# tprodanov/locityper

Hardware: AMD Instinct MI355X
Metric: reads/s through the whole genotyping path (scored + prefiltered + default solver scheme); reads_scored_per_s and genotypes_solved_per_s give the two halves (higher is better)
Workload: dtype f64

## Files before the change

locityper_amd/csrc/lcty_api.hip:

```cpp
#include <algorithm>
#include <cmath>
#include <memory>
#include <numeric>

#include "lcty_objects.hpp"

using namespace lcty;

namespace lcty {
static thread_local std::string g_last_error;
thread_local hipStream_t tl_stream = nullptr;
void set_last_error(const std::string& msg) { g_last_error = msg; }
}

hipEvent_t lcty_ctx::get_event() {
    hipEvent_t e;
    if (!event_pool.empty()) { e = event_pool.back(); event_pool.pop_back(); return e; }
    LCTY_HIP(hipEventCreate(&e));
    return e;
}

void lcty_ctx::fold_oldest(lcty::KernelTimer& t, size_t count) {
    count = std::min(count, t.pending.size());
    for (size_t i = 0; i < count; i++) {
        float ms = 0.f;
        LCTY_HIP(hipEventSynchronize(t.pending[i].second));
        LCTY_HIP(hipEventElapsedTime(&ms, t.pending[i].first, t.pending[i].second));
        t.total_ms += ms; t.launches++;
        event_pool.push_back(t.pending[i].first); event_pool.push_back(t.pending[i].second);
    }
    t.pending.erase(t.pending.begin(), t.pending.begin() + static_cast<std::ptrdiff_t>(count));
}

extern "C" {

int32_t lcty_ctx_set_knob(lcty_ctx* ctx, const char* name, int64_t value) {
    return guarded([&] {
        if (!ctx || !name) fail(LCTY_ERR_INVALID_INPUT, "null argument");
        static const char* const known[] = {"transfer_levels", "transfer_scratch_mb", "transfer_waves", "transfer_cap_new", "transfer_arena",
                                            "depth_table_start", "solve_budget_mb", "solve_chains_per_wave", "solve_extra_start", "solve_lds_weights",
                                            "anneal_lds_weights", "contig_info_slide", "gather_chunk_mb", "prefilter_gram", "prefilter_gram_cols",
                                            "prefilter_gram_levels", "comm_fail_at", "score_lean", "arena_cap_pct", "exact_threads", "host_threads",
                                            "score_lean_keep", "score_lean_two", "queue_early_head", "db_chunk_cols", "basis_batch_words",
                                            "align_batch_pairs", "align_hash_bits", "align_dp_cells", "align_match_budget", "align_cigar_store_mb", "pafvcf_hash_bits", "pafvcf_table_mb",
                                            "genome_max_bases", "sample_bam_hash_bits", "sample_bam_max_slice_bytes", "sample_bam_inflate",
                                            "bgzf_deflate", "bgzf_deflate_max_bytes", "aln_bam_max_slice_bytes", "vcf_max_slice_bytes", "fastx_window_bytes", "fastx_window_limit", "recruit_blocks",
                                            "recruited_init_units", "recruited_max_bytes",
#ifdef LCTY_DIAG
                                            "solve_stats", "queue_trace", "map_trace", "exact_trace", "solve_greedy_form", "solve_anneal_timing", "score_timing",
                                            "solve_init_tiles", "transfer_phases", "genome_scan_form",
#endif
                                            nullptr};
        bool ok = false;
        for (const char* const* k = known; *k; k++) ok |= strcmp(*k, name) == 0;
        if (!ok) fail(LCTY_ERR_INVALID_INPUT, "unknown knob '%s'", name);
        if (strcmp(name, "bgzf_deflate") == 0 && value != 0 && value != 1) fail(LCTY_ERR_INVALID_INPUT, "bgzf_deflate = %lld (0: host, 1: device)", static_cast<long long>(value));
        if (value < 0) ctx->knobs.erase(name); else ctx->knobs[name] = value;
    });
}

int32_t lcty_ctx_set_path(lcty_ctx* ctx, const char* name, const char* path) {
    return guarded([&] {
        if (!ctx || !name) fail(LCTY_ERR_INVALID_INPUT, "null argument");
        if (strcmp(name, "exact_dump") != 0) fail(LCTY_ERR_INVALID_INPUT, "unknown path '%s'", name);
        ctx->exact_dump_path = path ? path : "";
    });
}

const char* lcty_last_error(void) { return g_last_error.c_str(); }
const char* lcty_version(void) { return "locityper_hip 0.1.0 (gfx950)"; }

int32_t lcty_device_count(void) {
    int n = 0;
    if (hipGetDeviceCount(&n) != hipSuccess) { (void)hipGetLastError(); return 0; }
    return n;
}

int32_t lcty_ctx_create(int32_t device_id, lcty_ctx** out) {
    return guarded([&] {
        if (!out) fail(LCTY_ERR_INVALID_INPUT, "null argument");
        int n = 0;
        if (hipGetDeviceCount(&n) != hipSuccess || n == 0) {
            (void)hipGetLastError();
            fail(LCTY_ERR_RUNTIME, "no HIP device is visible: liblocityper_hip has no CPU fallback");
        }
        if (device_id < 0 || device_id >= n) fail(LCTY_ERR_INVALID_INPUT, "device %d out of range (0..%d)", device_id, n - 1);
        auto c = std::unique_ptr<lcty_ctx>(new lcty_ctx());
        c->device = device_id;
        LCTY_HIP(hipSetDevice(device_id));
// ... 327 lines not shown
```

locityper_amd/csrc/lcty_solve_device.hpp:

```cpp
#pragma once
#include "lcty_objects.hpp"

namespace lcty {

constexpr uint32_t MAXP = 4;
constexpr uint32_t NONE32S = 0xFFFFFFFFu;
constexpr uint32_t MID_NONE24 = 0xFFFFFFu;
constexpr uint64_t WINDOW_KEY_XOR = 0xD1B54A32D192ED03ull;
constexpr uint64_t INIT_KEY_XOR = 0x8CB92BA72F3D8DD7ull;

struct FastDiv {
    uint32_t d, m, s1, s2;
    __host__ static FastDiv make(uint32_t d) {
        FastDiv f{d, 0, 0, 0};
        uint32_t l = 0;
        while ((1ull << l) < d) l++;
        f.m = static_cast<uint32_t>(((1ull << 32) * ((1ull << l) - d)) / d + 1);
        f.s1 = l < 1 ? l : 1; f.s2 = l > 0 ? l - 1 : 0;
        return f;
    }
    __device__ __forceinline__ uint32_t div(uint32_t n) const {
        const uint32_t t = __umulhi(m, n);
        return (t + ((n - t) >> s1)) >> s2;
    }
// ... 124 lines not shown
static_assert(sizeof(InitGroup) == 48 && INIT_TILE_R <= 8, "InitGroup layout");
struct InitPlan {
    std::vector<InitGroup> groups; std::vector<InitChainP> chains;
    uint32_t T = 0, R = 0;
    size_t lds = 0;
};

inline void set_rec_list(SolveView& V, uint64_t n_reads) {
    V.seg_reads = static_cast<uint32_t>(((n_reads + INIT_SEGS - 1) / INIT_SEGS + 63) / 64 * 64);
    if (V.seg_reads == 0) V.seg_reads = 64;
    V.rstride = static_cast<uint64_t>(INIT_SEGS) * V.seg_reads;
}
inline size_t init_chain_lds(uint32_t wstride) { return ((static_cast<size_t>(wstride) * 4 + 15) & ~static_cast<size_t>(15)) + 256 * 8 + 64; }

template <typename... P, typename... A>
void launch_lds(lcty_ctx* ctx, int timer, void (*kernel)(P...), dim3 grid, dim3 block, size_t lds, hipStream_t s, const A&... args) {
    if (lds > 48 * 1024)
        LCTY_HIP(hipFuncSetAttribute(reinterpret_cast<const void*>(kernel), hipFuncAttributeMaxDynamicSharedMemorySize, static_cast<int>(lds)));
    auto go = [&] { hipLaunchKernelGGL(kernel, grid, block, lds, s, args...); };
    if (timer < 0) go();
    else ctx->timed(timer, go, s);
    LCTY_HIP(hipGetLastError());
}

void check_solver(const lcty_solver* solver);

void ensure_solver_tables(lcty_reads* reads);
void ensure_depth_table(lcty_locus* loc, uint64_t want);
void build_depth_table_into(const lcty_locus* loc, uint32_t depth, DevBuf<double>& out, hipStream_t s);
bool solver_lds_fits(uint32_t wstride);
struct InitHost {
    const uint16_t* genotypes; const uint64_t* seeds; const uint16_t* row_of; const lcty_locus* loc; uint32_t n_cus;
    uint32_t lds_budget;
};
void plan_init_groups(const SolveView& V, const InitHost& H, uint32_t nch, InitPlan& plan);
void launch_init(lcty_ctx* ctx, const SolveView& V, uint32_t nch, size_t lds_init, hipStream_t s, const InitHost* host, lcty_ctx::SolveWorkspace& ws,
                 InitPlan& plan);
void launch_greedy_chains(lcty_ctx* ctx, SolveView& V, uint32_t nch, hipStream_t stream, lcty_ctx::SolveWorkspace& ws);
void launch_anneal(lcty_ctx* ctx, const SolveView& V, uint32_t nch, hipStream_t s);
void launch_pause(hipStream_t s);
void launch_store_cur(ChainRec* recs, const uint32_t* words, uint64_t n, hipStream_t s);
void launch_pack_rows_count(uint64_t n, const LocCell* table, uint64_t ngp, uint32_t n_good, const uint16_t* alleles, uint32_t n_rows,
                            unsigned long long* total, hipStream_t s);
void launch_pack_rows(uint64_t n, const LocCell* table, const uint32_t* table_ext, const double* table_unm, uint64_t ngp, uint32_t n_good,
                      const uint16_t* alleles, uint32_t n_rows, const PairAlnDev* pa, LocEntry* cells, uint64_t out_stride, PairAlnDev* extras,
                      unsigned long long* cursor, hipStream_t s);
void launch_place_rows(uint64_t n, const LocEntry* cells, uint64_t in_stride, uint32_t n_good, uint32_t n_rows, uint32_t ext_base, LocCell* full,
                       uint32_t* full_ext, double* full_unm, bool write_unm, uint64_t full_stride, uint64_t first, hipStream_t s);
void launch_pad_rows(uint64_t n, LocCell* full, uint32_t* full_ext, double* full_unm, uint64_t full_stride, uint64_t from, uint32_t n_rows, hipStream_t s);
void launch_count_unexplained(uint32_t blocks, const uint8_t* status, const double* unmapped, const double* matrix, uint64_t n_pairs, uint32_t A,
                              const uint16_t* ids, uint32_t ploidy, unsigned long long* out, hipStream_t s);
void launch_read_nw(const SolveView& V, uint32_t* nw, hipStream_t s);
void launch_assignment_counts(const SolveView& V, const uint32_t* nw, const uint64_t* read_off, uint16_t* counts, hipStream_t s);

}
```

locityper_amd/csrc/lcty_solve_host.hip:

```cpp
#include <algorithm>
#include <atomic>
#include <cmath>
#include <exception>
#include <memory>
#include <numeric>
#include <future>
#include <thread>
#include <type_traits>

#include "lcty_exact.hpp"
#include "lcty_solve_device.hpp"

using namespace lcty;

namespace {

double students_t_cdf(double freedom, double x) {
    if (std::isinf(freedom)) return 0.5 * std::erfc(-x / std::sqrt(2.0));
    const double h = freedom / (freedom + x * x);
    const double ib = 0.5 * math::beta_reg(freedom / 2.0, 0.5, h);
    return x <= 0.0 ? ib : 1.0 - ib;
}

double compare_two(double mean1, double var1, uint32_t att1, double mean2, double var2, uint32_t att2) {
// ... 18 lines not shown

void sort_by_mean(const double* lik_mean, uint64_t* ixs, uint64_t n) {
    std::sort(ixs, ixs + n, [&](uint64_t a, uint64_t b) {
        if (lik_mean[a] != lik_mean[b]) return lik_mean[a] > lik_mean[b];
        return a < b;
    });
}

double ln_sum(const double* v, size_t n) {
    if (n == 0) return -std::numeric_limits<double>::infinity();
    if (n == 1) return v[0];
    double m = -std::numeric_limits<double>::infinity();
    for (size_t i = 0; i < n; i++) m = std::fmax(m, v[i]);
    if (std::isinf(m)) return m;
    double s = 0.0;
    for (size_t i = 0; i < n; i++) s += std::exp(v[i] - m);
    return m + std::log(s);
}

}

namespace {

struct StageRunner {
    lcty_reads* reads; lcty_ctx* ctx; lcty_locus* loc;
    SolveView V{};
    uint64_t n_gt; uint32_t ploidy, attempts;
    size_t lds_init = 0;
    uint64_t gt_per_batch = 1, depth_cap = 2;
    uint32_t lane;
    hipStream_t stream;
    lcty_ctx::SolveWorkspace& ws;
    InitPlan init_plan;
    InitHost init_host{nullptr, nullptr, nullptr, nullptr, 0, 0};
    const RowGatherer* gathered_rows = nullptr;

    StageRunner(lcty_reads* r, const uint16_t* genotypes, uint64_t n_gt_, uint32_t ploidy_, const lcty_solver* solver, uint32_t attempts_,
                const uint64_t* chain_seeds, uint32_t lane_ = 0, const RowGatherer* gathered = nullptr)
        : reads(r), n_gt(n_gt_), ploidy(ploidy_), attempts(attempts_), lane(lane_), ws(check_args(r, genotypes, solver, chain_seeds, lane_)) {
        if (!reads->scored) fail(LCTY_ERR_INVALID_INPUT, "lcty_score_reads has not been called on this batch");
        if (ploidy == 0 || ploidy > MAXP) fail(LCTY_ERR_UNSUPPORTED, "the device solver handles ploidy 1..%u", MAXP);
        if (attempts == 0) fail(LCTY_ERR_INVALID_INPUT, "At least one attempt is required for each stage");
        check_solver(solver);
        ctx = reads->ctx; loc = reads->locus; gathered_rows = gathered;
        ctx->activate();
        stream = lane ? ctx->side_stream() : ctx->stream;
        reads->check_device_error(stream);
        const uint32_t A = loc->n_alleles;
        for (uint64_t i = 0; i < n_gt * ploidy; i++)
            if (genotypes[i] >= A) fail(LCTY_ERR_INVALID_INPUT, "genotype refers to allele %u >= %u", genotypes[i], A);
        if (n_gt * attempts >= 0x7FFFFFFFull) fail(LCTY_ERR_UNSUPPORTED, "too many chains in one stage");
        if (!gathered) ensure_solver_tables(reads);
        reads->stat_chains = reads->stat_iterations = reads->stat_accepted = 0;
        const uint64_t n_good = gathered ? gathered->n_good : reads->n_good_cached, ngp = gathered ? gathered->ngp : reads->ngp;
        uint32_t min_w = 0xFFFFFFFFu;
        for (uint32_t a = 0; a < A; a++) min_w = std::min(min_w, std::max(loc->n_windows[a], 1u));
        depth_cap = 2 * n_good + 2;
        uint64_t first_width = std::min<uint64_t>(4 * n_good / min_w + 64, depth_cap);
        if (ctx->knob("depth_table_start", 0) > 0)
            first_width = static_cast<uint64_t>(ctx->knob("depth_table_start", 0));
        ensure_depth_table(loc, first_width);

        V.by_window = FastDiv::make(loc->bg.window); V.by_tweak = FastDiv::make(2 * static_cast<uint32_t>(loc->prm.tweak) + 1);
        V.A = A; V.window = loc->bg.window; V.left_padding = loc->left_padding; V.tweak = static_cast<uint32_t>(loc->prm.tweak);
        V.min_weight = loc->prm.min_weight; V.prob_diff = loc->prm.prob_diff;
        V.depth_contrib = 1.0 + loc->prm.lik_skew; V.aln_contrib = 1.0 - loc->prm.lik_skew;
        V.n_windows = loc->d_n_windows.p; V.reg_start = loc->d_reg_start.p; V.allele_len = loc->d_allele_len.p;
// ... 255 lines not shown
            std::vector<uint32_t> words(V.rstride);
            for (size_t k = 0; k < gn; k++) {
                Held& h = held[k];
                const uint32_t c0 = todo[g0 + k];
                for (uint64_t j = 0; j < V.rstride; j++) words[j] = h.recs[j].rp_cur;
                for (uint32_t i = 0; i < h.model.n; i++) words[h.place[i]] = (words[h.place[i]] & 0xFFFFFFu) | (static_cast<uint32_t>(h.res.assign[i]) << 24);
                d_words.upload(words.data(), V.rstride, s);
                const uint32_t c1 = shared_model ? std::min(c0 + attempts, nch) : c0 + 1;
                for (uint32_t c = c0; c < c1; c++) {
                    if (nnt[c] != h.model.n) fail(LCTY_ERR_RUNTIME, "exact solver: the attempts of a genotype without a tweak differ in their models");
                    launch_store_cur(V.recs + static_cast<uint64_t>(c) * V.rstride, d_words.p, V.rstride, s);
                    liks[c] = pri[c / attempts] + h.res.value;
                    parts[4ull * c] = h.res.aln_lik; parts[4ull * c + 1] = h.res.depth_lik; parts[4ull * c + 2] = static_cast<double>(h.res.nodes); parts[4ull * c + 3] = 0.0;
                }
                LCTY_HIP(hipStreamSynchronize(s));
            }
            LCTY_HIP(hipStreamSynchronize(s));
        }
        ws.liks.upload(liks.data(), nch, s);
        ws.parts.upload(parts.data(), 4ull * nch, s);
        LCTY_HIP(hipStreamSynchronize(s));
    }

    template <typename F>
    void run(const uint16_t* genotypes, const double* priors, const uint64_t* chain_seeds, F&& after_batch) {
        hipStream_t s = stream;
        std::vector<double> liks(gt_per_batch * attempts);
        for (uint64_t g0 = 0; g0 < n_gt;) {
            const uint64_t ng = std::min(gt_per_batch, n_gt - g0), nch = ng * attempts;
            bool smaller_batches = false;
            upload_genotypes(genotypes + g0 * ploidy, ng);
            ws.seeds.upload(chain_seeds + g0 * attempts, nch, s);
            init_host = InitHost{genotypes + g0 * ploidy, chain_seeds + g0 * attempts, gathered_rows ? gathered_rows->row_of.data() : nullptr, loc,
                                 static_cast<uint32_t>(ctx->props.multiProcessorCount), lane == 1 ? 32u * 1024u : 0u};
            if (priors) ws.pri.upload(priors + g0, ng, s);
            V.priors = priors ? ws.pri.p : nullptr;
            for (;;) {
                V.lut = loc->d_lut_ext.p; V.lut_depth = loc->lut_ext_depth; V.lut_shift = static_cast<uint32_t>(__builtin_ctz(loc->lut_ext_depth));
                launch(static_cast<uint32_t>(nch));
                uint32_t ovf[2] = {0, 0};
                ws.ovf.download(ovf, 2, s);
                ws.liks.download(liks.data(), nch, s);
                LCTY_HIP(hipStreamSynchronize(s));
                if (!ovf[0]) {
                    std::vector<double> parts(4 * nch);
                    ws.parts.download(parts.data(), 4 * nch, s);
                    LCTY_HIP(hipStreamSynchronize(s));
                    double sum = 0, mx = 0, mn = 1e300, acc = 0;
                    for (uint64_t c = 0; c < nch; c++) {
                        const double it = parts[4 * c + 2];
                        sum += it; mx = std::max(mx, it); mn = std::min(mn, it); acc += parts[4 * c + 3];
                    }
                    reads->stat_chains += nch; reads->stat_iterations += static_cast<uint64_t>(sum);
                    reads->stat_accepted += static_cast<uint64_t>(acc);
                    if (ctx->diag_knob("solve_stats", 0))
                        fprintf(stderr, "[lcty solve] chains=%llu iterations mean=%.0f min=%.0f max=%.0f accepted mean=%.0f lut_depth=%u\n",
                                static_cast<unsigned long long>(nch), sum / nch, mn, mx, acc / nch, loc->lut_ext_depth);
                    break;
                }
                if (ovf[0] == 2) fail(LCTY_ERR_UNSUPPORTED, "a read pair with more than 255 possible locations on one genotype (or 2^24 further locations in a chain)");
                if (ovf[0] == 3) fail(LCTY_ERR_RUNTIME, "annealing kernel: the staging wavefront and the chain lost each other");
                ws.ovf.zero(s);
                if (ovf[0] == 4) {
                    if (ovf[1] >= (1u << 24)) fail(LCTY_ERR_UNSUPPORTED, "2^24 or more further locations in one chain");
                    ws.extra_cap = std::min<uint32_t>(std::max<uint32_t>(ovf[1] + ovf[1] / 8 + 64, 2 * ws.extra_cap), (1u << 24) - 1);
                    const uint64_t before = gt_per_batch;
                    plan_batches();
// ... 694 lines not shown
```

locityper_amd/csrc/lcty_solve_kernels.hip:

```cpp
#include <algorithm>
#include <cmath>
#include <type_traits>
#include <vector>

#include "lcty_solve_device.hpp"

namespace lcty {


__global__ __launch_bounds__(256) void build_loc_table_kernel(const uint32_t* __restrict__ good_ix, uint32_t n_good, uint64_t ngp,
                                                              uint32_t A, const uint32_t* __restrict__ pa_idx,
                                                              const uint64_t* __restrict__ pa_off, const PairAlnDev* __restrict__ pa,
                                                              const double* __restrict__ unmapped, LocCell* __restrict__ table,
                                                              uint32_t* __restrict__ table_ext, double* __restrict__ table_unm,
                                                              uint32_t* __restrict__ err) {
    __shared__ LocCell tile[32][33];
    __shared__ uint32_t tile_ext[32][33];
    const uint32_t g0 = blockIdx.x * 32, c0 = blockIdx.y * 32;
    const uint32_t tx = threadIdx.x & 31u, ty = threadIdx.x >> 5;
    if (blockIdx.y == 0 && threadIdx.x < 32) {
        const uint32_t g = g0 + threadIdx.x;
        if (g < ngp) table_unm[g] = g < n_good ? unmapped[good_ix[g]] : 0.0;
    }
    for (uint32_t i = ty; i < 32; i += 8) {
// ... 388 lines not shown
    __syncthreads();
    const uint32_t ex_total = seg_cnt[4];
    if (tid == 0) {
        if (ex_total > V.extra_cap) { atomicMax(V.overflow, 4u); atomicMax(V.overflow + 1, ex_total); }
        if (ex_total >= (1u << 24)) atomicMax(V.overflow, 2u);
    }
    for (uint32_t s = 128; s > 0; s >>= 1) {
        if (tid < s) red[tid] += red[tid + s];
        __syncthreads();
    }
    uint32_t* gdepth = V.c_depth + static_cast<uint64_t>(chain) * V.wstride;
    for (uint32_t w = tid; w < G.total_w; w += 256) gdepth[w] = depth[w];
    if (tid == 0) {
        uint32_t* cum = V.c_seg + static_cast<uint64_t>(chain) * 4;
        uint32_t run = 0;
        for (uint32_t k = 0; k < INIT_SEGS; k++) { cum[k] = run; run += seg_cnt[k]; }
        V.c_aln[chain] = red[0]; V.c_nnt[chain] = run; V.c_totw[chain] = G.total_w;
    }
}

__device__ __forceinline__ uint64_t counter_fin(uint64_t z) {
    z = (z ^ (z >> 30)) * 0xbf58476d1ce4e5b9ull;
    z = (z ^ (z >> 27)) * 0x94d049bb133111ebull;
    return z ^ (z >> 31);
}
constexpr uint64_t GOLDEN64 = 0x9e3779b97f4a7c15ull;
typedef uint32_t u32x4_t __attribute__((ext_vector_type(4)));
__device__ __forceinline__ void store_16(uint4* p, uint4 v) {
    u32x4_t x; x.x = v.x; x.y = v.y; x.z = v.z; x.w = v.w;
    __builtin_nontemporal_store(x, reinterpret_cast<u32x4_t*>(p));
}
__host__ __device__ inline size_t init_tile_lds(uint32_t T, uint32_t R, uint32_t wstride) {
    const size_t depth = (static_cast<size_t>(T) * wstride * 4 + 15) & ~static_cast<size_t>(15);
    return depth + static_cast<size_t>(T) * 256 * 8 + 4ull * R * 64 * 16 + static_cast<size_t>(T) * 4 * 8 + static_cast<size_t>(T) * 4 * 5 + 64;
}

__device__ __forceinline__ void init_tile_deferred(const SolveView& V, const InitChainP* __restrict__ cp, uint32_t T, uint32_t* depth, double* aln_def,
                                                   uint32_t* ex_cnt, unsigned long long* queue, uint32_t head, uint32_t n, uint32_t wave, uint32_t lane, bool random_start) {
    double add = 0.0;
    uint32_t my_c = 0xFFFFFFFFu;
    if (lane < n) {
        const unsigned long long packed = __hip_atomic_load(&queue[(head + lane) & (INIT_TILE_Q - 1)], __ATOMIC_RELAXED, __HIP_MEMORY_SCOPE_WORKGROUP);
        const uint2 item = make_uint2(static_cast<uint32_t>(packed), static_cast<uint32_t>(packed >> 32));
        const uint32_t c = item.x >> 24, rp = item.x & 0xFFFFFFu, slot = item.y;
        const InitChainP P = cp[c];
        Geno<2> G;
        G.id[0] = P.id0; G.id[1] = P.id1; G.row[0] = P.row0; G.row[1] = P.row1; G.shift[0] = P.shift0; G.shift[1] = P.shift1;
        G.reg_start[0] = P.rs0; G.reg_start[1] = P.rs1; G.reg_end[0] = P.re0; G.reg_end[1] = P.re1; G.total_w = P.total_w;
        Locs<2> L;
        locs_init<2>(L, V, rp, G);
        if (L.nw > 255) atomicMax(V.overflow, 2u);
        uint32_t a0 = 0;
        if (L.nw > 1 && random_start)
            a0 = static_cast<uint32_t>(__umul64hi(counter_u64(P.seed ^ INIT_KEY_XOR, rp), static_cast<uint64_t>(L.nw)));
        const uint32_t nloc = min(L.nw, 255u), n_extra = nloc > 2 ? nloc - 2u : 0u;
        uint32_t eix = 0;
        if (n_extra) eix = atomicAdd(&ex_cnt[c], n_extra);
        const bool room = static_cast<uint64_t>(eix) + n_extra <= V.extra_cap;
        ExtraLoc* extra = V.extra + static_cast<uint64_t>(P.chain) * V.extra_cap;
        ChainRec rec; rec.rp_cur = rp | (a0 << 24); rec.meta = nloc | (eix << 8);
        rec.lp0 = rec.lp1 = 0.0; rec.win0 = rec.win1 = 0;
        LocIter<2> it; it.start(L);
        LocOut o;
        for (uint32_t t = 0; t < nloc && it.next(L, V, o); t++) {
            uint32_t wa, wb;
            loc_windows(V, G, o, P.seed, rp, t, &wa, &wb);
            const uint32_t win = wa | (wb << 16);
// ... 2 lines not shown
            else if (room) { ExtraLoc e; e.lp = o.lp; e.win = win; e._pad = 0; extra[eix + t - 2] = e; }
            if (t == a0) {
                atomicAdd(&depth[static_cast<size_t>(c) * V.wstride + wa], 1u);
                atomicAdd(&depth[static_cast<size_t>(c) * V.wstride + wb], 1u);
                add = o.lp;
                my_c = c;
            }
        }
        if (L.nw > 1) V.recs[static_cast<uint64_t>(P.chain) * V.rstride + static_cast<uint64_t>(wave) * V.seg_reads + slot] = rec;
    }
    for (uint32_t c = 0; c < T; c++) {
        unsigned long long m = __ballot(my_c == c);
        if (!m) continue;
        double acc = aln_def[c * 4 + wave];
        while (m) {
            const int l = __ffsll(static_cast<long long>(m)) - 1;
            acc += __hiloint2double(__builtin_amdgcn_readlane(__double2hiint(add), l), __builtin_amdgcn_readlane(__double2loint(add), l));
            m &= m - 1;
        }
        if (lane == 0) aln_def[c * 4 + wave] = acc;
    }
}

__global__ __launch_bounds__(256) void solve_init_tile_kernel(const SolveView V, const InitGroup* __restrict__ groups, const InitChainP* __restrict__ chains,
                                                             unsigned long long* lists, const uint32_t T_max, const uint32_t R_max) {
    extern __shared__ __align__(16) uint8_t smem[];
    const uint32_t tid = threadIdx.x, lane = tid & 63u, wave = __builtin_amdgcn_readfirstlane(tid >> 6);
    const InitGroup& grp = groups[blockIdx.x];
    const uint32_t T = grp.n_chains, R = grp.n_rows;
    const InitChainP* __restrict__ cp = chains + grp.first;
    const uint32_t W = V.wstride;
    uint32_t* depth = reinterpret_cast<uint32_t*>(smem);
    size_t at = (static_cast<size_t>(T_max) * W * 4 + 15) & ~static_cast<size_t>(15);
    double* aln = reinterpret_cast<double*>(smem + at); at += static_cast<size_t>(T_max) * 256 * 8;
    uint4* stage = reinterpret_cast<uint4*>(smem + at) + static_cast<size_t>(wave) * R_max * 64; at += 4ull * R_max * 64 * 16;
    unsigned long long* queue = lists + (static_cast<size_t>(blockIdx.x) * 4 + wave) * INIT_TILE_Q;
    double* aln_def = reinterpret_cast<double*>(smem + at); at += static_cast<size_t>(T_max) * 4 * 8;
    uint32_t* ex_cnt = reinterpret_cast<uint32_t*>(smem + at); at += static_cast<size_t>(T_max) * 4;
    uint32_t* seg_cnt = reinterpret_cast<uint32_t*>(smem + at);

    for (uint32_t c = 0; c < T; c++) {
        const InitChainP P = cp[c];
        double* ww = V.c_ww + static_cast<uint64_t>(P.chain) * W;
        uint8_t* wgc = V.c_gc + static_cast<uint64_t>(P.chain) * W;
        uint32_t* wuc = V.n_wk ? V.c_uc + static_cast<uint64_t>(P.chain) * W : nullptr;
        for (uint32_t w = tid; w < P.total_w; w += 256) {
            depth[c * W + w] = 0;
            double weight = 0.0; uint32_t g = 0, uc = V.n_wk - 1;
            if (w >= 2) {
                const bool second = w >= P.shift1;
                const uint32_t allele = second ? P.id1 : P.id0, sh = second ? P.shift1 : P.shift0, rs = second ? P.rs1 : P.rs0;
                const uint32_t start = rs + (w - sh) * V.window, end = start + V.window;
                const uint32_t left = min(V.tweak, start), right = min(V.tweak, V.allele_len[allele] - end);
                const uint64_t r = counter_u64(P.seed ^ WINDOW_KEY_XOR, w);
                const int64_t off = -static_cast<int64_t>(left) + static_cast<int64_t>(__umul64hi(r, static_cast<uint64_t>(left + right + 1)));
                const uint32_t wstart = static_cast<uint32_t>(static_cast<int64_t>(start) + off);
                const uint32_t i = V.ci_off[allele] + (wstart > V.left_padding ? wstart - V.left_padding : 0u);
                weight = V.win_weight[i];
                g = V.gc[i];
                if (wuc) uc = V.uniq_cnt[i] | (static_cast<uint32_t>(V.compl_cnt[i]) << 16);
                if (weight < V.min_weight || weight < 1e-7) { weight = 0.0; g = 0; uc = V.n_wk - 1; }
            }
            ww[w] = weight; wgc[w] = static_cast<uint8_t>(g);
            if (wuc) wuc[w] = uc;
        }
        aln[c * 256 + tid] = 0.0;
        if (tid < 4) aln_def[c * 4 + tid] = 0.0;
        if (tid == 0) ex_cnt[c] = 0;
    }
    __syncthreads();

    const bool random_start = V.solver.kind == LCTY_SOLVER_ANNEAL || (V.solver.kind == LCTY_SOLVER_GREEDY && !V.solver.best_start);
    const uint32_t seg_lo = min(wave * V.seg_reads, V.n_good), seg_hi = min(seg_lo + V.seg_reads, V.n_good);
    uint64_t row_at[INIT_TILE_R];
#pragma unroll
    for (uint32_t r = 0; r < INIT_TILE_R; r++) row_at[r] = static_cast<uint64_t>(grp.row[r < R ? r : 0]) * V.ngp;
    const uint4* __restrict__ table = reinterpret_cast<const uint4*>(V.table);
    uint4 nxt[INIT_TILE_R]; double nxt_unm = 0.0;
#pragma unroll
    for (uint32_t r = 0; r < INIT_TILE_R; r++) nxt[r] = make_uint4(0, 0, 0, 0);
    if (seg_lo + lane < seg_hi) {
#pragma unroll
        for (uint32_t r = 0; r < INIT_TILE_R; r++) if (r < R) nxt[r] = table[row_at[r] + seg_lo + lane];
        nxt_unm = V.table_unm[seg_lo + lane];
    }
    uint32_t n_recs_all = 0;
    uint32_t qn = 0, qhead = 0;
    for (uint32_t base = seg_lo; base < seg_hi; base += 64) {
        const uint32_t rp = base + lane;
        const bool in = rp < seg_hi;
#pragma unroll
        for (uint32_t r = 0; r < INIT_TILE_R; r++) if (r < R) stage[r * 64 + lane] = nxt[r];
        const double unm = nxt_unm;
        if (rp + 64 < seg_hi) {
#pragma unroll
            for (uint32_t r = 0; r < INIT_TILE_R; r++) if (r < R) nxt[r] = table[row_at[r] + rp + 64];
            nxt_unm = V.table_unm[rp + 64];
        }
        const uint64_t zbase = ((static_cast<uint64_t>(rp) << 16) + 1ull) * GOLDEN64;
        const uint64_t abase = (static_cast<uint64_t>(rp) + 1ull) * GOLDEN64;
        for (uint32_t c = 0; c < T; c++) {
            const InitChainP P = cp[c];
            const uint4 qa = stage[P.ia * 64 + lane], qb = stage[P.ib * 64 + lane];
            const double aln_before = aln[c * 256 + tid];
            const double lpA = __hiloint2double(static_cast<int>(qa.y), static_cast<int>(qa.x));
            const double lpB = __hiloint2double(static_cast<int>(qb.y), static_cast<int>(qb.x));
            const uint32_t rawA = qa.z >> 24, rawB = qb.z >> 24;
            const double thresh = fmax(fmax(lpA, lpB), unm) - V.prob_diff;
            const bool kA = in && rawA != 0 && lpA >= thresh, kB = in && rawB != 0 && lpB >= thresh, kU = in && unm >= thresh;
            const bool multi = (kA && rawA > 1) || (kB && rawB > 1);
            const uint32_t nw = (kA ? 1u : 0u) + (kB ? 1u : 0u) + (kU ? 1u : 0u);
            bool nontrivial = nw > 1;
            if (__any(multi && nw == 1)) {
                if (multi && nw == 1) {
                    const uint32_t ext = V.table_ext[static_cast<uint64_t>(kA ? P.row0 : P.row1) * V.ngp + rp];
                    nontrivial = V.pa[ext].ln_prob >= thresh;
                }
            }
            const unsigned long long nt_mask = __ballot(nontrivial);
            const uint32_t before = __builtin_amdgcn_readlane(n_recs_all, c);
            const uint32_t slot = before + static_cast<uint32_t>(__popcll(nt_mask & ((1ull << lane) - 1ull)));
            {
                const uint32_t after = __builtin_amdgcn_readfirstlane(before + static_cast<uint32_t>(__popcll(nt_mask)));
                uint32_t m0_was;
                asm volatile("s_mov_b32 %1, m0\n\ts_mov_b32 m0, %3\n\tv_writelane_b32 %0, %2, m0\n\ts_mov_b32 m0, %1"
                             : "+v"(n_recs_all), "=&s"(m0_was) : "s"(after), "s"(c));
            }
            const unsigned long long mm = __ballot(multi);
            if (mm) {
                if (multi)
                    __hip_atomic_store(&queue[(qhead + qn + static_cast<uint32_t>(__popcll(mm & ((1ull << lane) - 1ull)))) & (INIT_TILE_Q - 1)],
                                       static_cast<unsigned long long>(rp | (c << 24)) | (static_cast<unsigned long long>(slot) << 32), __ATOMIC_RELAXED,
                                       __HIP_MEMORY_SCOPE_WAVEFRONT);
                qn += static_cast<uint32_t>(__popcll(mm));
            }
            const bool BgtA = lpB > lpA, UgtA = unm > lpA, UgtB = unm > lpB;
            const uint32_t posA = ((kB && BgtA) ? 1u : 0u) + ((kU && UgtA) ? 1u : 0u);
// ... 2 lines not shown
            if (V.tweak) {
                const uint64_t z0 = P.seed + zbase;
                const uint64_t rA = counter_fin(z0 + (posA == 0 ? 0ull : posA == 1 ? GOLDEN64 : 2ull * GOLDEN64));
                const uint64_t rB = counter_fin(z0 + (posB == 0 ? 0ull : posB == 1 ? GOLDEN64 : 2ull * GOLDEN64));
                tA1 = V.by_tweak.mod(static_cast<uint32_t>(rA >> 32)); tA2 = V.by_tweak.mod(static_cast<uint32_t>(rA));
                tB1 = V.by_tweak.mod(static_cast<uint32_t>(rB >> 32)); tB2 = V.by_tweak.mod(static_cast<uint32_t>(rB));
            }
            auto window_ix = [&](uint32_t mid, bool none, uint32_t tw, uint32_t rs, uint32_t re, uint32_t sh) -> uint32_t {
                const uint32_t m = mid + tw;
                uint32_t q = V.by_window.div(m - rs) + sh;
                asm volatile("" : "+v"(q));
                const uint32_t inside = (rs <= m && m < re) ? q : 1u;
                return none ? 0u : inside;
            };
            const uint32_t midA1 = qa.z & MID_NONE24, midB1 = qb.z & MID_NONE24;
            const uint32_t winA = window_ix(midA1, midA1 == MID_NONE24, tA1, P.rs0, P.re0, P.shift0) |
                                  (window_ix(qa.w, qa.w == NONE32S, tA2, P.rs0, P.re0, P.shift0) << 16);
            const uint32_t winB = window_ix(midB1, midB1 == MID_NONE24, tB1, P.rs1, P.re1, P.shift1) |
                                  (window_ix(qb.w, qb.w == NONE32S, tB2, P.rs1, P.re1, P.shift1) << 16);
            const bool a_0 = kA && posA == 0, b_0 = kB && posB == 0, a_1 = kA && posA == 1, b_1 = kB && posB == 1, a_2 = kA && posA == 2, b_2 = kB && posB == 2;
            const double lp0 = a_0 ? lpA : (b_0 ? lpB : unm), lp1 = a_1 ? lpA : (b_1 ? lpB : unm), lp2 = a_2 ? lpA : (b_2 ? lpB : unm);
            const uint32_t win0 = a_0 ? winA : (b_0 ? winB : 0u), win1 = a_1 ? winA : (b_1 ? winB : 0u), win2 = a_2 ? winA : (b_2 ? winB : 0u);
            uint32_t a0 = 0;
            double lps = lp0; uint32_t wins = win0;
            if (random_start) {
                const uint64_t r = counter_fin((P.seed ^ INIT_KEY_XOR) + abase);
                a0 = nw > 1 ? static_cast<uint32_t>(__umul64hi(r, static_cast<uint64_t>(nw))) : 0u;
                lps = a0 == 0 ? lp0 : (a0 == 1 ? lp1 : lp2); wins = a0 == 0 ? win0 : (a0 == 1 ? win1 : win2);
            }
            const bool fast = !multi && nw != 0;
            if (fast) {
                atomicAdd(&depth[c * W + (wins & 0xFFFFu)], 1u);
                atomicAdd(&depth[c * W + (wins >> 16)], 1u);
                aln[c * 256 + tid] = aln_before + lps;
            }
            uint32_t eix = 0;
            if (fast && nw == 3) {
                eix = atomicAdd(&ex_cnt[c], 1u);
                if (eix < V.extra_cap) {
                    ExtraLoc e; e.lp = lp2; e.win = win2; e._pad = 0;
                    V.extra[static_cast<uint64_t>(P.chain) * V.extra_cap + eix] = e;
                }
            }
            if (fast && nw > 1) {
                uint4* dst = reinterpret_cast<uint4*>(V.recs + static_cast<uint64_t>(P.chain) * V.rstride + static_cast<uint64_t>(wave) * V.seg_reads + slot);
                store_16(dst, make_uint4(rp | (a0 << 24), nw | (eix << 8), static_cast<uint32_t>(__double2loint(lp0)), static_cast<uint32_t>(__double2hiint(lp0))));
                store_16(dst + 1, make_uint4(static_cast<uint32_t>(__double2loint(lp1)), static_cast<uint32_t>(__double2hiint(lp1)), win0, win1));
            }
        }
        const bool last = base + 64 >= seg_hi;
        if (qn >= 64 || (last && qn)) {
            __builtin_amdgcn_fence(__ATOMIC_RELEASE, "workgroup");
            __builtin_amdgcn_wave_barrier();
            __builtin_amdgcn_fence(__ATOMIC_ACQUIRE, "workgroup");
            while (qn >= 64 || (last && qn)) {
                const uint32_t n = min(qn, 64u);
                init_tile_deferred(V, cp, T, depth, aln_def, ex_cnt, queue, qhead, n, wave, lane, random_start);
                qhead = (qhead + n) & (INIT_TILE_Q - 1); qn -= n;
            }
        }
    }
    if (lane < T) seg_cnt[lane * 4 + wave] = n_recs_all;
    __syncthreads();
    for (uint32_t c = 0; c < T; c++) {
        const InitChainP P = cp[c];
        const uint32_t ex_total = ex_cnt[c];
        if (tid == 0) {
            if (ex_total > V.extra_cap) { atomicMax(V.overflow, 4u); atomicMax(V.overflow + 1, ex_total); }
            if (ex_total >= (1u << 24)) atomicMax(V.overflow, 2u);
        }
        uint32_t* gdepth = V.c_depth + static_cast<uint64_t>(P.chain) * W;
        for (uint32_t w = tid; w < P.total_w; w += 256) gdepth[w] = depth[c * W + w];
        if (wave == 0) {
            double v = (aln[c * 256 + lane] + aln[c * 256 + 64 + lane]) + (aln[c * 256 + 128 + lane] + aln[c * 256 + 192 + lane]);
            for (int o = 32; o > 0; o >>= 1) v += __shfl_xor(v, o);
            v += (aln_def[c * 4] + aln_def[c * 4 + 1]) + (aln_def[c * 4 + 2] + aln_def[c * 4 + 3]);
            if (lane == 0) {
                uint32_t* cum = V.c_seg + static_cast<uint64_t>(P.chain) * 4;
                uint32_t run = 0;
                for (uint32_t k = 0; k < INIT_SEGS; k++) { cum[k] = run; run += seg_cnt[c * 4 + k]; }
                V.c_aln[P.chain] = v; V.c_nnt[P.chain] = run; V.c_totw[P.chain] = P.total_w;
            }
        }
    }
}

struct PairGather { int32_t c[2]; uint32_t dmax[2]; double weight[2], vnew[2], vold[2]; };
__device__ __forceinline__ double pair_term(const PairGather& g, int i, uint32_t* deepest) {
    const bool live = g.c[i] != 0 && g.weight[i] != 0.0;
    *deepest = max(*deepest, live ? g.dmax[i] : 0u);
    return live ? g.weight[i] * g.vnew[i] - g.weight[i] * g.vold[i] : 0.0;
}

__device__ __forceinline__ double lut_at(const double* lut, uint32_t index) {
    return *reinterpret_cast<const double*>(reinterpret_cast<const char*>(lut) + (index << 3));
}
constexpr uint32_t DEPTH_MASK = 0x1FFFFFFu;
struct WinGathered {
    static constexpr bool WEIGHTS_LAST = false;
    uint32_t* wd;
    const double* ww;
    struct Word { uint32_t word; };
    __device__ __forceinline__ Word at(uint32_t w) const { return Word{wd[w]}; }
    __device__ __forceinline__ uint32_t depth(Word x) const { return x.word & DEPTH_MASK; }
    __device__ __forceinline__ uint32_t gc(Word x) const { return x.word >> 25; }
    __device__ __forceinline__ double weight(Word x, uint32_t w) const { return ww[w]; }
};
// ... 1078 lines not shown
    if (want > 0) {
        const uint32_t forced = want >= 6 ? 10u : want == 5 ? 12u : static_cast<uint32_t>(64 / std::min<int64_t>(want, 4));
        if (forced >= S) lpc = forced;
    }
    const bool lw = V.n_wk != 0 && 2 * static_cast<uint64_t>(V.n_good) + 2 <= LW_DEPTH_MASK && ctx->knob("solve_lds_weights", 1) != 0;
    while (lpc < 64 && greedy_lds(lpc, V, lw) > 80 * 1024) lpc = lpc < 16 ? 16 : lpc * 2;
    auto go = [&](auto tag) {
        constexpr uint32_t L = decltype(tag)::value;
        if (lw) launch_greedy<L, true>(ctx, V, nch, stream); else launch_greedy<L, false>(ctx, V, nch, stream);
    };
    const bool timed_form = lpc == 12 && lw && (ctx->diag_knob("solve_greedy_form", 0) & 32) != 0;
    const size_t n_waves = (static_cast<size_t>(nch) + 4) / 5 + 2;
    V.dbg = nullptr;
    if (timed_form) { ws.dbg.ensure(12 * n_waves); ws.dbg.zero(stream); V.dbg = ws.dbg.p; }
    if (lpc == 10) go(std::integral_constant<uint32_t, 10>{});
    else if (lpc == 12) go(std::integral_constant<uint32_t, 12>{});
    else if (lpc == 16) go(std::integral_constant<uint32_t, 16>{});
    else if (lpc == 32) go(std::integral_constant<uint32_t, 32>{});
    else go(std::integral_constant<uint32_t, 64>{});
    if (timed_form) {
        std::vector<double> d(12 * n_waves);
        ws.dbg.download(d.data(), d.size(), stream);
        LCTY_HIP(hipStreamSynchronize(stream));
        double sum[12] = {0}; size_t used = 0;
        for (size_t w = 0; w < n_waves; w++) if (d[12 * w + 6] > 0) { used++; for (int k = 0; k < 12; k++) sum[k] += d[12 * w + k] / d[12 * w + 6]; }
        if (used) fprintf(stderr, "[lcty greedy phases] %zu wavefronts; clock ticks per iteration: candidates+requests %.0f (waiting for the further locations %.0f, current location %.0f, its pair %.0f, first alternative %.0f), ext+sample+record request %.0f, wait+score %.0f, row best %.0f, move %.0f; loop total %.0f; a round for the second alternative in %.3f of the iterations\n",
                          used, sum[0] / used, sum[11] / used, sum[8] / used, sum[9] / used, sum[10] / used, sum[1] / used, sum[2] / used, sum[3] / used, sum[4] / used, sum[5] / used, sum[7] / used);
    }
}

bool solver_lds_fits(uint32_t wstride) {
    return !(static_cast<size_t>(wstride) * 12 + sizeof(AnnealRing) + 128 > 160 * 1024 || wstride > 65535);
}
void plan_init_groups(const SolveView& V, const InitHost& H, uint32_t nch, InitPlan& plan) {
    plan.groups.clear(); plan.chains.clear(); plan.T = plan.R = 0; plan.lds = 0;
    const uint32_t attempts = V.attempts, ng = (nch + attempts - 1) / attempts, A = V.A;
    uint32_t T_cap = INIT_TILE_T;
    const size_t lds_budget = H.lds_budget ? H.lds_budget : 80 * 1024;
    while (T_cap > 1 && init_tile_lds(T_cap, std::min(INIT_TILE_R, T_cap + 1), V.wstride) > lds_budget) T_cap--;
    const uint64_t per_cu = std::max<uint64_t>(1, std::min<uint64_t>(160 * 1024 / init_tile_lds(T_cap, std::min(INIT_TILE_R, T_cap + 1), V.wstride), 4));
    const uint64_t places = per_cu * std::max(1u, H.n_cus);
    T_cap = static_cast<uint32_t>(std::max<uint64_t>(1, std::min<uint64_t>(T_cap, (nch + places - 1) / places)));
    const uint32_t R_cap = std::min(INIT_TILE_R, T_cap + 1);
    std::vector<uint32_t> deg(A, 0), rank(A, 0), order(A);
    for (uint32_t g = 0; g < ng; g++) { deg[H.genotypes[2 * g]]++; deg[H.genotypes[2 * g + 1]]++; }
    for (uint32_t a = 0; a < A; a++) order[a] = a;
    std::stable_sort(order.begin(), order.end(), [&](uint32_t x, uint32_t y) { return deg[x] > deg[y]; });
    for (uint32_t r = 0; r < A; r++) rank[order[r]] = r;
    std::vector<uint32_t> gts(ng);
    std::vector<uint64_t> key(ng);
    for (uint32_t g = 0; g < ng; g++) {
        const uint32_t ra = rank[H.genotypes[2 * g]], rb = rank[H.genotypes[2 * g + 1]];
        const uint64_t u = std::min(ra, rb), v = std::max(ra, rb);
        key[g] = ((u / 2) << 48) | ((v / 4) << 32) | (u << 16) | v;
        gts[g] = g;
    }
    std::sort(gts.begin(), gts.end(), [&](uint32_t x, uint32_t y) { return key[x] != key[y] ? key[x] < key[y] : x < y; });
    auto row_of = [&](uint32_t allele) -> uint32_t { return H.row_of ? H.row_of[allele] : allele; };
    struct Unit { uint32_t gi, a0, n; };
    struct Proto { std::vector<Unit> units; uint32_t n_chains = 0, n_rows = 0; uint32_t row[8] = {0, 0, 0, 0, 0, 0, 0, 0}; };
    std::vector<Proto> protos;
    Proto cur;
    auto close = [&] { if (cur.n_chains) protos.push_back(cur); cur = Proto{}; };
    auto fresh_rows = [&](const Proto& p, uint32_t r0, uint32_t r1) -> uint32_t {
        bool h0 = false, h1 = false;
        for (uint32_t r = 0; r < p.n_rows; r++) { h0 |= p.row[r] == r0; h1 |= p.row[r] == r1; }
        return (h0 ? 0u : 1u) + ((h1 || r1 == r0) ? 0u : 1u);
    };
    auto add_rows = [&](Proto& p, uint32_t r0, uint32_t r1) {
        for (uint32_t x : {r0, r1}) {
            bool have = false;
            for (uint32_t r = 0; r < p.n_rows; r++) have |= p.row[r] == x;
            if (!have) p.row[p.n_rows++] = x;
        }
    };
// ... 36 lines not shown
        for (const Unit& u : p.units) {
            const uint32_t id0 = H.genotypes[2 * u.gi], id1 = H.genotypes[2 * u.gi + 1];
            const uint32_t row0 = row_of(id0), row1 = row_of(id1);
            uint32_t ia = 0, ib = 0;
            for (uint32_t r = 0; r < p.n_rows; r++) { if (p.row[r] == row0) ia = r; if (p.row[r] == row1) ib = r; }
            const uint32_t nw0 = H.loc->n_windows[id0], nw1 = H.loc->n_windows[id1];
            for (uint32_t k = 0; k < u.n; k++) {
                const uint32_t chain = u.gi * attempts + u.a0 + k;
                if (chain >= nch) break;
                InitChainP P{};
                P.seed = H.seeds[chain]; P.chain = chain; P.ia = ia; P.ib = ib; P.row0 = row0; P.row1 = row1; P.id0 = id0; P.id1 = id1;
                P.shift0 = 2; P.rs0 = H.loc->reg_start[id0]; P.re0 = P.rs0 + nw0 * V.window;
                P.shift1 = 2 + nw0; P.rs1 = H.loc->reg_start[id1]; P.re1 = P.rs1 + nw1 * V.window;
                P.total_w = 2 + nw0 + nw1;
                plan.chains.push_back(P);
                g.n_chains++;
            }
        }
        if (!g.n_chains) continue;
        plan.T = std::max(plan.T, g.n_chains); plan.R = std::max(plan.R, g.n_rows);
        plan.groups.push_back(g);
    }
    plan.lds = init_tile_lds(plan.T, plan.R, V.wstride);
}

void launch_init(lcty_ctx* ctx, const SolveView& V, uint32_t nch, size_t lds_init, hipStream_t s, const InitHost* host, lcty_ctx::SolveWorkspace& ws,
                 InitPlan& plan) {
    if (V.ploidy == 2 && host && nch && ctx->diag_knob("solve_init_tiles", 1) != 0) {
        plan_init_groups(V, *host, nch, plan);
        const size_t gb = plan.groups.size() * sizeof(InitGroup), cb = plan.chains.size() * sizeof(InitChainP);
        if (ctx->diag_knob("solve_stats", 0)) {
            uint64_t rows = 0; uint32_t hist[INIT_TILE_T + 1] = {0};
            for (const InitGroup& g : plan.groups) { rows += g.n_rows; hist[g.n_chains]++; }
            fprintf(stderr, "[lcty solve] initialisation: %u chains in %zu groups (largest %u chains, %u rows; %.2f rows per chain; LDS %zu B); groups of 1..%u chains:",
                    nch, plan.groups.size(), plan.T, plan.R, static_cast<double>(rows) / nch, plan.lds, INIT_TILE_T);
            for (uint32_t t = 1; t <= INIT_TILE_T; t++) fprintf(stderr, " %u", hist[t]);
            fprintf(stderr, "\n");
        }
        const size_t lb = plan.groups.size() * 4 * INIT_TILE_Q * sizeof(unsigned long long);
        ws.init_plan.ensure_slack(gb + cb + lb);
        LCTY_HIP(hipMemcpyAsync(ws.init_plan.p, plan.groups.data(), gb, hipMemcpyHostToDevice, s));
        LCTY_HIP(hipMemcpyAsync(ws.init_plan.p + gb, plan.chains.data(), cb, hipMemcpyHostToDevice, s));
        launch_lds(ctx, V.solver.kind == LCTY_SOLVER_ANNEAL ? LCTY_K_SOLVE_INIT_ANNEAL : LCTY_K_SOLVE_INIT, solve_init_tile_kernel,
                   dim3(static_cast<uint32_t>(plan.groups.size())), dim3(256), plan.lds, s, V, reinterpret_cast<const InitGroup*>(ws.init_plan.p),
                   reinterpret_cast<const InitChainP*>(ws.init_plan.p + gb), reinterpret_cast<unsigned long long*>(ws.init_plan.p + gb + cb), plan.T, plan.R);
        return;
    }
    switch (V.ploidy) {
        case 1: launch_init_p<1>(ctx, V, nch, lds_init, s); break;
        case 2: launch_init_p<2>(ctx, V, nch, lds_init, s); break;
        case 3: launch_init_p<3>(ctx, V, nch, lds_init, s); break;
        default: launch_init_p<4>(ctx, V, nch, lds_init, s); break;
    }
}
void launch_pause(hipStream_t s) { hipLaunchKernelGGL(pause_kernel, dim3(1), dim3(64), 0, s, 8u); }
void launch_store_cur(ChainRec* recs, const uint32_t* words, uint64_t n, hipStream_t s) {
    hipLaunchKernelGGL(store_cur_kernel, dim3(static_cast<uint32_t>((n + 255) / 256)), dim3(256), 0, s, recs, words, n);
    LCTY_HIP(hipGetLastError());
}
void launch_pack_rows_count(uint64_t n, const LocCell* table, uint64_t ngp, uint32_t n_good, const uint16_t* alleles, uint32_t n_rows,
                            unsigned long long* total, hipStream_t s) {
    hipLaunchKernelGGL(pack_rows_count_kernel, dim3(static_cast<uint32_t>((n + 255) / 256)), dim3(256), 0, s, table, ngp, n_good, alleles, n_rows, total);
    LCTY_HIP(hipGetLastError());
}
void launch_pack_rows(uint64_t n, const LocCell* table, const uint32_t* table_ext, const double* table_unm, uint64_t ngp, uint32_t n_good,
                      const uint16_t* alleles, uint32_t n_rows, const PairAlnDev* pa, LocEntry* cells, uint64_t out_stride, PairAlnDev* extras,
                      unsigned long long* cursor, hipStream_t s) {
    hipLaunchKernelGGL(pack_rows_kernel, dim3(static_cast<uint32_t>((n + 255) / 256)), dim3(256), 0, s, table, table_ext, table_unm, ngp, n_good, alleles,
// ... 37 lines not shown
```

Before: 2.718 million.

## Keep init-tile alignment sums in registers and overlay LDS to fit three workgroups per CU

The init tile kernel now accumulates per-chain alignment log-probabilities in a per-thread register array instead of LDS. It writes them to LDS only once at the end, into space shared with the staging buffer. This shrinks the LDS footprint. The default LDS budget drops from 80 KB to about a third of 160 KB, rounded to the allocation granule, so three workgroups can be resident per CU, and the per-CU count now accounts for that granularity. A new knob can select two per CU or skip the occupancy-based chain cap. The risks are more register pressure from the switch-indexed accumulator array and fewer chains per tile.

```diff
diff --git a/locityper_amd/csrc/lcty_api.hip b/locityper_amd/csrc/lcty_api.hip
--- a/locityper_amd/csrc/lcty_api.hip
+++ b/locityper_amd/csrc/lcty_api.hip
@@ -38,7 +38,7 @@
     return guarded([&] {
         if (!ctx || !name) fail(LCTY_ERR_INVALID_INPUT, "null argument");
         static const char* const known[] = {"transfer_levels", "transfer_scratch_mb", "transfer_waves", "transfer_cap_new", "transfer_arena",
-                                            "depth_table_start", "solve_budget_mb", "solve_chains_per_wave", "solve_extra_start", "solve_lds_weights",
+                                            "depth_table_start", "solve_budget_mb", "solve_chains_per_wave", "solve_extra_start", "solve_lds_weights", "solve_init_layout",
                                             "anneal_lds_weights", "contig_info_slide", "gather_chunk_mb", "prefilter_gram", "prefilter_gram_cols",
                                             "prefilter_gram_levels", "comm_fail_at", "score_lean", "arena_cap_pct", "exact_threads", "host_threads",
                                             "score_lean_keep", "score_lean_two", "queue_early_head", "db_chunk_cols", "basis_batch_words",
@@ -55,6 +55,7 @@
         for (const char* const* k = known; *k; k++) ok |= strcmp(*k, name) == 0;
         if (!ok) fail(LCTY_ERR_INVALID_INPUT, "unknown knob '%s'", name);
         if (strcmp(name, "bgzf_deflate") == 0 && value != 0 && value != 1) fail(LCTY_ERR_INVALID_INPUT, "bgzf_deflate = %lld (0: host, 1: device)", static_cast<long long>(value));
+        if (strcmp(name, "solve_init_layout") == 0 && value > 2) fail(LCTY_ERR_INVALID_INPUT, "solve_init_layout = %lld (0: the plan's, 1: two workgroups per CU, 2: three)", static_cast<long long>(value));
         if (value < 0) ctx->knobs.erase(name); else ctx->knobs[name] = value;
     });
 }
diff --git a/locityper_amd/csrc/lcty_solve_device.hpp b/locityper_amd/csrc/lcty_solve_device.hpp
--- a/locityper_amd/csrc/lcty_solve_device.hpp
+++ b/locityper_amd/csrc/lcty_solve_device.hpp
@@ -180,6 +180,7 @@
 struct InitHost {
     const uint16_t* genotypes; const uint64_t* seeds; const uint16_t* row_of; const lcty_locus* loc; uint32_t n_cus;
     uint32_t lds_budget;
+    uint32_t layout;
 };
 void plan_init_groups(const SolveView& V, const InitHost& H, uint32_t nch, InitPlan& plan);
 void launch_init(lcty_ctx* ctx, const SolveView& V, uint32_t nch, size_t lds_init, hipStream_t s, const InitHost* host, lcty_ctx::SolveWorkspace& ws,
diff --git a/locityper_amd/csrc/lcty_solve_host.hip b/locityper_amd/csrc/lcty_solve_host.hip
--- a/locityper_amd/csrc/lcty_solve_host.hip
+++ b/locityper_amd/csrc/lcty_solve_host.hip
@@ -74,7 +74,7 @@
     hipStream_t stream;
     lcty_ctx::SolveWorkspace& ws;
     InitPlan init_plan;
-    InitHost init_host{nullptr, nullptr, nullptr, nullptr, 0, 0};
+    InitHost init_host{nullptr, nullptr, nullptr, nullptr, 0, 0, 0};
     const RowGatherer* gathered_rows = nullptr;
 
     StageRunner(lcty_reads* r, const uint16_t* genotypes, uint64_t n_gt_, uint32_t ploidy_, const lcty_solver* solver, uint32_t attempts_,
@@ -396,7 +396,7 @@
             upload_genotypes(genotypes + g0 * ploidy, ng);
             ws.seeds.upload(chain_seeds + g0 * attempts, nch, s);
             init_host = InitHost{genotypes + g0 * ploidy, chain_seeds + g0 * attempts, gathered_rows ? gathered_rows->row_of.data() : nullptr, loc,
-                                 static_cast<uint32_t>(ctx->props.multiProcessorCount), lane == 1 ? 32u * 1024u : 0u};
+                                 static_cast<uint32_t>(ctx->props.multiProcessorCount), lane == 1 ? 32u * 1024u : 0u, static_cast<uint32_t>(ctx->knob("solve_init_layout", 0))};
             if (priors) ws.pri.upload(priors + g0, ng, s);
             V.priors = priors ? ws.pri.p : nullptr;
             for (;;) {
diff --git a/locityper_amd/csrc/lcty_solve_kernels.hip b/locityper_amd/csrc/lcty_solve_kernels.hip
--- a/locityper_amd/csrc/lcty_solve_kernels.hip
+++ b/locityper_amd/csrc/lcty_solve_kernels.hip
@@ -444,7 +444,8 @@
 }
 __host__ __device__ inline size_t init_tile_lds(uint32_t T, uint32_t R, uint32_t wstride) {
     const size_t depth = (static_cast<size_t>(T) * wstride * 4 + 15) & ~static_cast<size_t>(15);
-    return depth + static_cast<size_t>(T) * 256 * 8 + 4ull * R * 64 * 16 + static_cast<size_t>(T) * 4 * 8 + static_cast<size_t>(T) * 4 * 5 + 64;
+    const size_t strip = std::max<size_t>(4ull * R * 64 * 16, static_cast<size_t>(T) * 256 * 8);
+    return depth + strip + static_cast<size_t>(T) * 4 * 8 + static_cast<size_t>(T) * 4 * 5 + 64;
 }
 
 __device__ __forceinline__ void init_tile_deferred(const SolveView& V, const InitChainP* __restrict__ cp, uint32_t T, uint32_t* depth, double* aln_def,
@@ -513,8 +514,9 @@
     const uint32_t W = V.wstride;
     uint32_t* depth = reinterpret_cast<uint32_t*>(smem);
     size_t at = (static_cast<size_t>(T_max) * W * 4 + 15) & ~static_cast<size_t>(15);
-    double* aln = reinterpret_cast<double*>(smem + at); at += static_cast<size_t>(T_max) * 256 * 8;
-    uint4* stage = reinterpret_cast<uint4*>(smem + at) + static_cast<size_t>(wave) * R_max * 64; at += 4ull * R_max * 64 * 16;
+    double* hand = reinterpret_cast<double*>(smem + at);
+    uint4* stage = reinterpret_cast<uint4*>(smem + at) + static_cast<size_t>(wave) * R_max * 64;
+    at += max(4ull * R_max * 64 * 16, static_cast<unsigned long long>(T_max) * 256 * 8);
     unsigned long long* queue = lists + (static_cast<size_t>(blockIdx.x) * 4 + wave) * INIT_TILE_Q;
     double* aln_def = reinterpret_cast<double*>(smem + at); at += static_cast<size_t>(T_max) * 4 * 8;
     uint32_t* ex_cnt = reinterpret_cast<uint32_t*>(smem + at); at += static_cast<size_t>(T_max) * 4;
@@ -545,7 +547,6 @@
             ww[w] = weight; wgc[w] = static_cast<uint8_t>(g);
             if (wuc) wuc[w] = uc;
         }
-        aln[c * 256 + tid] = 0.0;
         if (tid < 4) aln_def[c * 4 + tid] = 0.0;
         if (tid == 0) ex_cnt[c] = 0;
     }
@@ -565,6 +566,9 @@
         for (uint32_t r = 0; r < INIT_TILE_R; r++) if (r < R) nxt[r] = table[row_at[r] + seg_lo + lane];
         nxt_unm = V.table_unm[seg_lo + lane];
     }
+    double acc[INIT_TILE_T];
+#pragma unroll
+    for (uint32_t k = 0; k < INIT_TILE_T; k++) acc[k] = 0.0;
     uint32_t n_recs_all = 0;
     uint32_t qn = 0, qhead = 0;
     for (uint32_t base = seg_lo; base < seg_hi; base += 64) {
@@ -583,7 +587,6 @@
         for (uint32_t c = 0; c < T; c++) {
             const InitChainP P = cp[c];
             const uint4 qa = stage[P.ia * 64 + lane], qb = stage[P.ib * 64 + lane];
-            const double aln_before = aln[c * 256 + tid];
             const double lpA = __hiloint2double(static_cast<int>(qa.y), static_cast<int>(qa.x));
             const double lpB = __hiloint2double(static_cast<int>(qb.y), static_cast<int>(qb.x));
             const uint32_t rawA = qa.z >> 24, rawB = qb.z >> 24;
@@ -652,7 +655,19 @@
             if (fast) {
                 atomicAdd(&depth[c * W + (wins & 0xFFFFu)], 1u);
                 atomicAdd(&depth[c * W + (wins >> 16)], 1u);
-                aln[c * 256 + tid] = aln_before + lps;
+            }
+            {
+                const double add = fast ? lps : 0.0;
+                switch (c) {
+                    case 0: acc[0] += add; break;
+                    case 1: acc[1] += add; break;
+                    case 2: acc[2] += add; break;
+                    case 3: acc[3] += add; break;
+                    case 4: acc[4] += add; break;
+                    case 5: acc[5] += add; break;
+                    case 6: acc[6] += add; break;
+                    default: acc[7] += add; break;
+                }
             }
             uint32_t eix = 0;
             if (fast && nw == 3) {
@@ -682,6 +697,9 @@
     }
     if (lane < T) seg_cnt[lane * 4 + wave] = n_recs_all;
     __syncthreads();
+#pragma unroll
+    for (uint32_t k = 0; k < INIT_TILE_T; k++) if (k < T) hand[k * 256 + tid] = acc[k];
+    __syncthreads();
     for (uint32_t c = 0; c < T; c++) {
         const InitChainP P = cp[c];
         const uint32_t ex_total = ex_cnt[c];
@@ -692,7 +710,7 @@
         uint32_t* gdepth = V.c_depth + static_cast<uint64_t>(P.chain) * W;
         for (uint32_t w = tid; w < P.total_w; w += 256) gdepth[w] = depth[c * W + w];
         if (wave == 0) {
-            double v = (aln[c * 256 + lane] + aln[c * 256 + 64 + lane]) + (aln[c * 256 + 128 + lane] + aln[c * 256 + 192 + lane]);
+            double v = (hand[c * 256 + lane] + hand[c * 256 + 64 + lane]) + (hand[c * 256 + 128 + lane] + hand[c * 256 + 192 + lane]);
             for (int o = 32; o > 0; o >>= 1) v += __shfl_xor(v, o);
             v += (aln_def[c * 4] + aln_def[c * 4 + 1]) + (aln_def[c * 4 + 2] + aln_def[c * 4 + 3]);
             if (lane == 0) {
@@ -1837,15 +1855,21 @@
 bool solver_lds_fits(uint32_t wstride) {
     return !(static_cast<size_t>(wstride) * 12 + sizeof(AnnealRing) + 128 > 160 * 1024 || wstride > 65535);
 }
+constexpr size_t INIT_LDS_GRANULE = 1280, INIT_LDS_THIRD = (160 * 1024 / INIT_LDS_GRANULE / 3) * INIT_LDS_GRANULE;
+static uint64_t init_groups_per_cu(size_t lds) {
+    const size_t granules = (lds + INIT_LDS_GRANULE - 1) / INIT_LDS_GRANULE;
+    return std::max<uint64_t>(1, std::min<uint64_t>(160 * 1024 / INIT_LDS_GRANULE / granules, 4));
+}
 void plan_init_groups(const SolveView& V, const InitHost& H, uint32_t nch, InitPlan& plan) {
     plan.groups.clear(); plan.chains.clear(); plan.T = plan.R = 0; plan.lds = 0;
     const uint32_t attempts = V.attempts, ng = (nch + attempts - 1) / attempts, A = V.A;
     uint32_t T_cap = INIT_TILE_T;
-    const size_t lds_budget = H.lds_budget ? H.lds_budget : 80 * 1024;
+    size_t lds_budget = H.layout == 1 ? 80 * 1024 : INIT_LDS_THIRD;
+    if (H.lds_budget) lds_budget = std::min<size_t>(lds_budget, H.lds_budget);
     while (T_cap > 1 && init_tile_lds(T_cap, std::min(INIT_TILE_R, T_cap + 1), V.wstride) > lds_budget) T_cap--;
-    const uint64_t per_cu = std::max<uint64_t>(1, std::min<uint64_t>(160 * 1024 / init_tile_lds(T_cap, std::min(INIT_TILE_R, T_cap + 1), V.wstride), 4));
+    const uint64_t per_cu = init_groups_per_cu(init_tile_lds(T_cap, std::min(INIT_TILE_R, T_cap + 1), V.wstride));
     const uint64_t places = per_cu * std::max(1u, H.n_cus);
-    T_cap = static_cast<uint32_t>(std::max<uint64_t>(1, std::min<uint64_t>(T_cap, (nch + places - 1) / places)));
+    if (!H.layout) T_cap = static_cast<uint32_t>(std::max<uint64_t>(1, std::min<uint64_t>(T_cap, (nch + places - 1) / places)));
     const uint32_t R_cap = std::min(INIT_TILE_R, T_cap + 1);
     std::vector<uint32_t> deg(A, 0), rank(A, 0), order(A);
     for (uint32_t g = 0; g < ng; g++) { deg[H.genotypes[2 * g]]++; deg[H.genotypes[2 * g + 1]]++; }
@@ -1948,8 +1972,11 @@
         if (ctx->diag_knob("solve_stats", 0)) {
             uint64_t rows = 0; uint32_t hist[INIT_TILE_T + 1] = {0};
             for (const InitGroup& g : plan.groups) { rows += g.n_rows; hist[g.n_chains]++; }
-            fprintf(stderr, "[lcty solve] initialisation: %u chains in %zu groups (largest %u chains, %u rows; %.2f rows per chain; LDS %zu B); groups of 1..%u chains:",
-                    nch, plan.groups.size(), plan.T, plan.R, static_cast<double>(rows) / nch, plan.lds, INIT_TILE_T);
+            int resident = 0;
+            LCTY_HIP(hipOccupancyMaxActiveBlocksPerMultiprocessor(&resident, reinterpret_cast<const void*>(solve_init_tile_kernel), 256, plan.lds));
+            fprintf(stderr, "[lcty solve] initialisation: %u chains in %zu groups (largest %u chains, %u rows; %.2f rows per chain; LDS %zu B, %llu workgroups per CU planned, %d by the runtime's count); groups of 1..%u chains:",
+                    nch, plan.groups.size(), plan.T, plan.R, static_cast<double>(rows) / nch, plan.lds,
+                    static_cast<unsigned long long>(init_groups_per_cu(plan.lds)), resident, INIT_TILE_T);
             for (uint32_t t = 1; t <= INIT_TILE_T; t++) fprintf(stderr, " %u", hist[t]);
             fprintf(stderr, "\n");
         }
```

Measured after the change: 2.631 million. -3.2%, worse.
